# fumiama/Retrieval-based-Voice-Conversion-WebUI

Hardware: AMD Instinct MI355X
Metric: real-time factor (audio-sec/wall-sec), 48 kHz v2, 10 s clips, retrieval + NSF-HiFi-GAN decode (higher is better)
Workload: dtype fp16 MFMA operands + fp16 inter-stage streams (ResBlock outputs, ups output of stages 1-3), fp32 accumulate / in-block residual; fp32 MFMA prefilter + fp64 verified IVF distances; 1 GPU; BASELINE configs[1]: v2/48k, 1 x 10 s clip(s) per GPU, T=1198 frames, 599 queries/clip, IVF 10000x768 nlist=256 nprobe=1 k=8 index_rate=0.75; hipgraph=True, index_blob_bytes=32376576, launcher=single process

## Files before the change

retrieval-based-voice-conversion-webui_amd/csrc/mfma_conv.hpp:

```cpp
#pragma once
#include <hip/hip_runtime.h>

#include <stdint.h>

namespace rvcmi {

using bf16x8 = __attribute__((ext_vector_type(8))) __bf16;
using f16x8 = __attribute__((ext_vector_type(8))) _Float16;
using f32x16 = __attribute__((ext_vector_type(16))) float;
using f32x4 = __attribute__((ext_vector_type(4))) float;

__device__ __forceinline__ float lrelu(float v, float slope) { return v > 0.f ? v : v * slope; }

__device__ __forceinline__ int item_rows(const int* __restrict__ lens, int b, int mul, int Lmax) {
    return lens ? max(min(Lmax, lens[b] * mul), min(Lmax, mul)) : Lmax;
}


template <typename OpT>
struct Op;
template <>
struct Op<__bf16> {
    using frag = bf16x8;
    static __device__ __forceinline__ f32x16 mfma(frag a, frag b, f32x16 c) {
// ... 134 lines not shown
}
template <typename OpT, int MI>
__device__ __forceinline__ void kconv_prefetch(typename Op<OpT>::frag (&A)[8][MI], __amdgpu_buffer_rsrc_t r, unsigned loff, unsigned ctb) {
#pragma unroll
    for (int kk = 0; kk < 8; ++kk)
#pragma unroll
        for (int mi = 0; mi < MI; ++mi) A[kk][mi] = weight_load<OpT>(r, loff + kk * 1024, mi * ctb);
}
template <typename OpT, int CIN, int MI, int NJ, int STRIDE, int JT0 = 0>
__device__ __forceinline__ void kconv(f32x16 (&acc)[MI][NJ], typename Op<OpT>::frag (&A)[8][MI], unsigned lds_row, __amdgpu_buffer_rsrc_t r,
                                      unsigned loff, unsigned ctb, int ntaps, int dstep) {
    using frag = typename Op<OpT>::frag;
    constexpr int CC = CIN / 16, GPT = CC / 8;
    static_assert(CIN % 128 == 0, "kconv: C_in must be a multiple of 128");
    static_assert(JT0 >= 0 && JT0 < NJ, "kconv: at least one column tile runs");
    constexpr int NJA = NJ - JT0;
    constexpr unsigned TS = 32u * STRIDE;
    auto ld = [](unsigned a) { return *(const __attribute__((address_space(3))) frag*)(size_t)a; };
    frag Bf[2][NJ];
#pragma unroll
    for (int jt = JT0; jt < NJ; ++jt) {
        Bf[0][jt] = ld(lds_row + jt * TS);
        __builtin_amdgcn_sched_barrier(0);
    }
    const unsigned dS = (unsigned)(dstep * STRIDE);
    const int ngroups = ntaps * GPT;
    const unsigned slast = (unsigned)(ngroups - 1) * 8192u;
    unsigned soff = ngroups > 1 ? 8192u : 0u;
    int gi = 0;
    for (int g = 0; g < ngroups; ++g) {
        const unsigned nrow = (gi + 1 == GPT) ? lds_row - (unsigned)((GPT - 1) * 256) + dS : lds_row + 256u;
        unsigned b0 = lds_row, b1 = nrow;
        asm volatile("" : "+v"(b0), "+v"(b1));
#pragma unroll
        for (int kk = 0; kk < 8; ++kk) {
#pragma unroll
            for (int mi = 0; mi < MI; ++mi)
#pragma unroll
                for (int jt = JT0; jt < NJ; ++jt) {
                    constexpr int NS = MI * NJA;
                    const int i = mi * NJA + jt - JT0;
                    acc[mi][jt] = Op<OpT>::mfma(A[kk][mi], Bf[kk & 1][jt], acc[mi][jt]);
                    if (i < NJA) Bf[(kk + 1) & 1][JT0 + i] = ld((kk < 7 ? b0 + (unsigned)((kk + 1) * 32) : b1) + (JT0 + i) * TS);
                    if (i >= NS - MI) A[kk][i - (NS - MI)] = weight_load<OpT>(r, loff + kk * 1024, soff + (unsigned)(i - (NS - MI)) * ctb);
                    __builtin_amdgcn_sched_barrier(0);
                }
        }
        lds_row = nrow;
        gi = (gi + 1 == GPT) ? 0 : gi + 1;
        soff = soff < slast ? soff + 8192u : soff;
    }
}

__host__ __device__ constexpr int mfma16_row(int n) { return n < 4 ? 2 * n : n < 12 ? 2 * n - 7 : 2 * n - 16; }
__host__ __device__ constexpr int mfma16_chunk(int q) { return ((q & 1) << 1) | (q >> 1); }
__device__ __forceinline__ unsigned mfma16_loff(int lane) {
    const int q = lane >> 4, n = lane & 15;
    return (unsigned)(((q & 1) * 64 + (q >> 1) * 32 + n) * 16);
}
template <typename OpT, int MI>
__device__ __forceinline__ void kconv16_prefetch(typename Op<OpT>::frag (&A)[8][MI], __amdgpu_buffer_rsrc_t r, unsigned loff, unsigned ctb) {
    static_assert(MI == 1, "kconv16: one 32-channel tile per wave");
#pragma unroll
    for (int s = 0; s < 4; ++s)
#pragma unroll
        for (int h = 0; h < 2; ++h) A[2 * s + h][0] = weight_load<OpT>(r, loff + s * 2048 + h * 256, 0);
}
template <typename OpT, int CIN, int MI, int NJ, int STRIDE, int JT0 = 0>
__device__ __forceinline__ void kconv16(f32x4 (&acc)[2 * MI][2 * NJ], typename Op<OpT>::frag (&A)[8][MI], unsigned lds_row,
                                        __amdgpu_buffer_rsrc_t r, unsigned loff, unsigned ctb, int ntaps, int dstep) {
    using frag = typename Op<OpT>::frag;
    constexpr int CC = CIN / 16, GPT = CC / 8, NT = 2 * NJ;
    static_assert(CIN % 128 == 0, "kconv16: C_in must be a multiple of 128");
    static_assert(MI == 1, "kconv16: one 32-channel tile per wave");
    static_assert(JT0 >= 0 && JT0 < NT, "kconv16: at least one column tile runs");
    constexpr unsigned TS = 16u * STRIDE;
    auto ld = [](unsigned a) { return *(const __attribute__((address_space(3))) frag*)(size_t)a; };
    frag Bf[NT];
#pragma unroll
    for (int jt = JT0; jt < NT; ++jt) {
        Bf[jt] = ld(lds_row + jt * TS);
        __builtin_amdgcn_sched_barrier(0);
    }
    const unsigned dS = (unsigned)(dstep * STRIDE);
    const int ngroups = ntaps * GPT;
    const unsigned slast = (unsigned)(ngroups - 1) * 8192u;
    unsigned soff = ngroups > 1 ? 8192u : 0u;
    int gi = 0;
    for (int g = 0; g < ngroups; ++g) {
        const unsigned nrow = (gi + 1 == GPT) ? lds_row - (unsigned)((GPT - 1) * 256) + dS : lds_row + 256u;
        unsigned b0 = lds_row, b1 = nrow;
        asm volatile("" : "+v"(b0), "+v"(b1));
#pragma unroll
        for (int s = 0; s < 4; ++s) {
#pragma unroll
            for (int jt = JT0; jt < NT; ++jt)
#pragma unroll
                for (int h = 0; h < 2; ++h) {
                    acc[h][jt] = Op<OpT>::mfma16(A[2 * s + h][0], Bf[jt], acc[h][jt]);
                    if (h == 1) Bf[jt] = ld((s < 3 ? b0 + (unsigned)((s + 1) * 64) : b1) + jt * TS);
                    if (jt == NT - 1) A[2 * s + h][0] = weight_load<OpT>(r, loff + s * 2048 + h * 256, soff);
                    __builtin_amdgcn_sched_barrier(0);
                }
        }
        lds_row = nrow;
        gi = (gi + 1 == GPT) ? 0 : gi + 1;
// ... 84 lines not shown
```

retrieval-based-voice-conversion-webui_amd/csrc/nsf.hip:

```cpp
#include <algorithm>
#include <atomic>
#include <cmath>
#include <functional>
#include <memory>
#include <string>
#include <unordered_map>

#include "common.hpp"
#include "nsf_source_kernels.hpp"
#include "conv_kernels.hpp"
#include "post_kernels.hpp"
#include "rb_pair_kernels.hpp"
#include "ups_kernels.hpp"
#include "rb_full_kernels.hpp"
#include "conv_pack.hpp"
#include "rb_stream.hpp"

namespace rvcmi {

struct Geom {
    int MI, NJ, WCO, TT;
};
static Geom conv_geom(int cout) {
    Geom g;
// ... 104 lines not shown
            const int ctiles = (s.cout + 31) / 32;
            std::vector<uint16_t> pk((size_t)ctiles * 512, 0);
            for (int ct = 0; ct < ctiles; ++ct)
                for (int lane = 0; lane < 64; ++lane)
                    for (int e = 0; e < 8; ++e) {
                        const int co = ct * 32 + (lane & 31), kk = 8 * (lane >> 5) + e;
                        if (co < s.cout && kk < s.nk) {
                            const float v = w[(size_t)co * s.nk + kk];
                            pk[(size_t)ct * 512 + lane * 8 + e] = op == RVCMI_OPERAND_BF16 ? f32_to_bf16(v) : f32_to_f16(v);
                        }
                    }
            upload(s.nz_k1_w, pk);
            s.nz_k1 = true;
        }
    }
    s.rb.resize(cfg->n_resblock_kernels);
    for (int j = 0; j < cfg->n_resblock_kernels; ++j) {
        const int n = i * cfg->n_resblock_kernels + j;
        const int k = cfg->resblock_kernel_sizes[j];
        const int nd = cfg->n_dilations[j];
        if (nd < 1 || nd > RVCMI_MAX_DIL || !(k & 1)) RVCMI_FAIL(RVCMI_ERR_INVALID, "bad resblock %d", j);
        s.rb[j].resize(nd);
        for (int m = 0; m < nd; ++m) {
            const int d = cfg->resblock_dilation_sizes[j][m];
            const std::string base = "resblocks." + std::to_string(n);
            const int C = s.cout;
            for (int which = 0; which < 2; ++which) {
                const std::string nm = base + (which ? ".convs2." : ".convs1.") + std::to_string(m);
                const float* w = wm.get(nm + ".weight", {C, C, k});
                const float* b = wm.get(nm + ".bias", {C});
                const int dil = which ? 1 : d;
                int nt = k, off = -((k * dil - dil) / 2);
                ConvLayer& L2 = which ? s.rb[j][m].second : s.rb[j][m].first;
                build_conv(L2, C, C, 1, &nt, &off, dil,
                           [=](int co, int ci, int, int tap) { return w[((size_t)co * C + ci) * k + tap]; }, b, op);
            }
        }
    }
}

static void nsf_create(const rvcmi_nsf_config* cfg, const rvcmi_tensor* weights, int n_weights, int device, int max_B,
                       int max_T, rvcmi_nsf** out) {
    if (!cfg || !out || (!weights && n_weights)) RVCMI_FAIL(RVCMI_ERR_INVALID, "null argument");
    if (cfg->n_ups < 1 || cfg->n_ups > RVCMI_MAX_UPS || cfg->n_resblock_kernels < 1 ||
        cfg->n_resblock_kernels > RVCMI_MAX_RB)
        RVCMI_FAIL(RVCMI_ERR_INVALID, "bad stage counts");
    if (cfg->operand < 0 || cfg->operand > 2) RVCMI_FAIL(RVCMI_ERR_INVALID, "bad operand type %d", cfg->operand);
    if (max_B < 1 || max_T < 1) RVCMI_FAIL(RVCMI_ERR_INVALID, "max_B/max_T must be positive");
    HIP_CHECK(hipSetDevice(device));
    set_lds_limits();
    rb_stream_prepare();

    std::unique_ptr<rvcmi_nsf> h(new rvcmi_nsf());
    h->opt.load_env({"RB_STREAM", "NO_RB_SPLIT", "POST_DMA", "POST_DBG", "RBF_PAD_TAP", "RBF32_TALL", "DBG", "Y_F16", "X0_F16", "X0_F16_NOSTREAM"});
    rb_stream_load_env(h->opt);
    h->cfg = *cfg;
    h->device = device;
    h->max_B = max_B;
    h->max_T = max_T;
    const int op = cfg->operand;
    WeightTable wm(weights, n_weights, "nsf_create");

    const int C0 = cfg->upsample_initial_channel, inter = cfg->inter_channels;
    h->C0 = C0;
    {
        const float* w = wm.get("conv_pre.weight", {C0, inter, 7});
        const float* b = wm.get("conv_pre.bias", {C0});
        int nt = 7, off = -3;
        build_conv(h->pre, inter, C0, 1, &nt, &off, 1,
                   [=](int co, int ci, int, int tap) { return w[((size_t)co * inter + ci) * 7 + tap]; }, b, op);
    }
    if (cfg->gin_channels) {
        const float* w = wm.get("cond.weight", {C0, cfg->gin_channels, 1});
        const float* b = wm.get("cond.bias", {C0});
        upload(h->cond_w, w, (size_t)C0 * cfg->gin_channels * sizeof(float));
        upload(h->cond_b, b, C0 * sizeof(float));
    }
    if (cfg->use_f0) {
        h->lin_w = wm.get("m_source.l_linear.weight", {1, 1})[0];
        h->lin_b = wm.get("m_source.l_linear.bias", {1})[0];
    }
    int upp = 1;
    for (int i = 0; i < cfg->n_ups; ++i) upp *= cfg->upsample_rates[i];
    h->upp = upp;

    h->stages.resize(cfg->n_ups);
    size_t S = (size_t)max_T * C0;
    long L = max_T;
    for (int i = 0; i < cfg->n_ups; ++i) {
        build_stage(h->stages[i], cfg, wm, i);
        L *= h->stages[i].u;
        S = std::max(S, (size_t)L * h->stages[i].cout);
    }
    h->c_last = C0 >> cfg->n_ups;
    {
        const float* w = wm.get("conv_post.weight", {1, h->c_last, 7});
        std::vector<float> wt((size_t)7 * h->c_last);
        for (int c = 0; c < h->c_last; ++c)
            for (int j = 0; j < 7; ++j) wt[(size_t)j * h->c_last + c] = w[(size_t)c * 7 + j];
        upload(h->post_w, wt);
    }
    if (h->c_last & 3) RVCMI_FAIL(RVCMI_ERR_INVALID, "last stage channel count %d", h->c_last);

    if (cfg->n_resblock_kernels > 3) RVCMI_FAIL(RVCMI_ERR_INVALID, "more than 3 resblock kernels per stage is unsupported");
    h->S = S * (size_t)max_B;
    const size_t fb = h->S * sizeof(float);
    h->P.alloc((size_t)max_B * max_T * C0 * sizeof(float));
// ... 145 lines not shown
    }
    if (smem > 160 * 1024) RVCMI_FAIL(RVCMI_ERR_INVALID, "upsampler LDS tile too large (%zu B)", smem);
    const int per_block = WV * a.vpw;
    dim3 grid((a.Lin + TQ - 1) / TQ, (a.nvt + per_block - 1) / per_block, B);
    {
        const int esz = a.out_half ? 2 : 4;
        const size_t ot = (size_t)TQ * a.u * ((size_t)a.cout * esz + 16);
        smem = (smem + 15) / 16 * 16;
        if (a.out_tr && grid.y == 1 && (a.cout * esz) % 16 == 0 && smem + ot <= 52 * 1024) {
            a.out_tr_off = (int)smem;
            smem += ot;
        } else {
            a.out_tr = 0;
        }
    }
    if (a.out_tw_off && !a.out_tr && a.out_half && nj == 1 && MI == 2 && a.cout % 64 == 0) {
        smem = (smem + 15) / 16 * 16;
        a.out_tw_off = (int)smem;
        smem += (size_t)4 * 32 * (MI * 64 + 16);
    } else {
        a.out_tw_off = 0;
    }
    if (nj == 4) hipLaunchKernelGGL((k_ups<OpT, CIN, MI, WV, 4>), grid, dim3(256), smem, st, a);
    else if (nj == 2) hipLaunchKernelGGL((k_ups<OpT, CIN, MI, WV, 2>), grid, dim3(256), smem, st, a);
    else hipLaunchKernelGGL((k_ups<OpT, CIN, MI, WV, 1>), grid, dim3(256), smem, st, a);
}
#define RVCMI_UPS_CASES(X, OpT) \
    X(OpT, 512, 2) X(OpT, 256, 2) X(OpT, 128, 2) X(OpT, 64, 1) X(OpT, 32, 1)
template <typename OpT>
static void launch_ups_t(const UpsArgs& a, int wv, int nj, int B, hipStream_t st) {
#define X(OpT_, CIN_, MI_)                                                        \
    if (a.cin == CIN_) {                                                          \
        if (wv == 4) return launch_ups_inst<OpT_, CIN_, MI_, 4>(a, nj, B, st);    \
        if (wv == 2) return launch_ups_inst<OpT_, CIN_, MI_, 2>(a, nj, B, st);    \
        return launch_ups_inst<OpT_, CIN_, MI_, 1>(a, nj, B, st);                 \
    }
    RVCMI_UPS_CASES(X, OpT)
#undef X
    RVCMI_FAIL(RVCMI_ERR_INVALID, "unsupported upsampler C_in %d", a.cin);
}
template <typename OpT>
static void set_lds_ups() {
#define Y(OpT_, CIN_, MI_, WV_, NJ_)                                                                                    \
    HIP_CHECK(hipFuncSetAttribute(reinterpret_cast<const void*>(&k_ups<OpT_, CIN_, MI_, WV_, NJ_>),                      \
                                  hipFuncAttributeMaxDynamicSharedMemorySize, 160 * 1024));
#define X(OpT_, CIN_, MI_)                                                                                              \
    Y(OpT_, CIN_, MI_, 4, 4) Y(OpT_, CIN_, MI_, 4, 2) Y(OpT_, CIN_, MI_, 4, 1) Y(OpT_, CIN_, MI_, 2, 4) Y(OpT_, CIN_, MI_, 2, 2)   \
    Y(OpT_, CIN_, MI_, 2, 1) Y(OpT_, CIN_, MI_, 1, 4) Y(OpT_, CIN_, MI_, 1, 2) Y(OpT_, CIN_, MI_, 1, 1)
    RVCMI_UPS_CASES(X, OpT)
#undef Y
#undef X
}

template <typename OpT, int C, int MI, int NJ, int NB, int OCC, int NWV>
static void launch_rbf(size_t smem, const RbFullArgs* ra, int tiles, int nj, int B, hipStream_t st) {
    auto kern = &k_rb_full<OpT, C, MI, NJ,  4, NB, OCC, NWV>;
    if (!ra) {
        HIP_CHECK(hipFuncSetAttribute(reinterpret_cast<const void*>(kern), hipFuncAttributeMaxDynamicSharedMemorySize, 160 * 1024));
        return;
    }
    hipLaunchKernelGGL(kern, dim3(tiles, nj, B), dim3(64 * NWV), smem, st, *ra);
}
struct RbFullClass {
    int C, rows, waves;
    int MI, NJ, NB, OCC;
    size_t lds_bytes;
    void (*launch[2])(size_t, const RbFullArgs*, int, int, int, hipStream_t);
};
#define RBF_CLASS(C_, MI_, NJ_, NB_, OCC_, NWV_, STAMP_B_)                                                                     \
    {C_, NWV_ * 32 * NJ_, NWV_, MI_, NJ_, NB_, OCC_,                                                                           \
     (size_t)(2 * (NWV_ * 32 * NJ_) + 2 * RBF_G + 2 * RBF_G2) * Tile<C_>::STRIDE + 3 * 2 * 32 * MI_ * 4 + STAMP_B_,            \
     {&launch_rbf<__bf16, C_, MI_, NJ_, NB_, OCC_, NWV_>, &launch_rbf<_Float16, C_, MI_, NJ_, NB_, OCC_, NWV_>}}
static constexpr RbFullClass RBF_CLASSES[] = {
    RBF_CLASS(64, 2, 2, 2, 2, 8, 512),
    RBF_CLASS(32, 1, 3, 3, 2, 4, 512),
    RBF_CLASS(16, 1, 3, 3, 2, 4, 512),
    RBF_CLASS(64, 2, 2, 3, 1, 4, 512),
    RBF_CLASS(32, 1, 2, 3, 2, 4, 512),
    RBF_CLASS(32, 1, 3, 3, 1, 8, 1024),
};
#undef RBF_CLASS
constexpr int RBF_SMALL_ROWS = 256, RBF_TALL_ROWS = 768;
static int rbf_default_rows(int C) { return C == 64 ? 512 : 384; }
static const RbFullClass* rbf_class(int C, int rows) {
    for (const RbFullClass& c : RBF_CLASSES)
        if (c.C == C && c.rows == rows) return &c;
    RVCMI_FAIL(RVCMI_ERR_INVALID, "fused resblock: no %d-row tile class for channel count %d", rows, C);
}
static void set_lds_rbf() {
    for (const RbFullClass& c : RBF_CLASSES)
        for (auto launch : c.launch) launch(c.lds_bytes, nullptr, 0, 0, 0, nullptr);
}

static int tri_mode(const rvcmi_nsf* h, const char* key) {
    const int v = h->opt.has(key) ? h->opt.geti(key, 2) : 2;
    return v == 0 || v == 1 ? v : 2;
}
static int rbf32_tall_mode(const rvcmi_nsf* h) { return tri_mode(h, "RBF32_TALL"); }
static int rb_stream_mode(const rvcmi_nsf* h) { return tri_mode(h, "RB_STREAM"); }

static bool y_f16(const rvcmi_nsf* h) {
    return h->cfg.operand != RVCMI_OPERAND_F32 && h->opt.geti("Y_F16", 1) != 0;
}

static void run_conv(rvcmi_nsf* h, const ConvLayer& L, ConvArgs a, int B, const char* name, hipStream_t st) {
    if (!a.cf_stride) a.cf_stride = a.Lin;
    a.cin = L.cin;
    a.cout = L.cout;
    a.bias = L.bias.as<float>();
    a.dstep = L.dstep;
    a.nphase = L.nphase;
    const int op = h->cfg.operand;
    int jsum = 0;
    for (int p = 0; p < L.nphase; ++p) {
        a.ph_in_off[p] = L.in_off[p];
        a.ph_ntaps[p] = L.ntaps[p];
        a.ph_w_off[p] = op == RVCMI_OPERAND_F32 ? L.f32_off[p] : L.pack_off[p];
        jsum += L.ntaps[p];
    }
    a.in_off = L.in_off[0];
    const double flops = L.flops_per_pos * (double)a.Lq * B;
    const size_t esz = op == RVCMI_OPERAND_F32 ? 4 : 2;
    double bytes = (double)B * a.Lin * L.cin * (a.in_mode == IN_OP_RAW ? esz : 4) +
                   (double)B * a.Lq * L.nphase * L.cout * (a.out_mode == OUT_ACT ? esz : 4) * (a.accumulate ? 2 : 1) +
                   (a.res ? (double)B * a.Lq * L.nphase * L.cout * 4 : 0) + (double)jsum * L.cin * L.cout * esz;
    if (op == RVCMI_OPERAND_F32) {
        a.w = L.w_f32.p;
        a.ntaps = L.ntaps[0];
        a.roff = 0;
        a.tile_rows = 0;
        const size_t n = (size_t)a.Lq * a.cout;
        dim3 grid((unsigned)((n + 255) / 256), L.nphase, B);
        h->prof.launch(name, flops, bytes, st, [&] { hipLaunchKernelGGL(k_conv_f32, grid, dim3(256), 0, st, a); });
    } else {
        Geom g = conv_geom(L.cout);
        int nj = 4;
        if (g.MI == 2 && g.WCO == 4 && (long)B * ((a.Lq + g.TT - 1) / g.TT) * ((L.cout + 255) / 256) * L.nphase < 128) {
            nj = 1;
            g.TT = 32;
        }
        a.w = L.w_pack.p;
        a.w_ct_stride = L.ct_stride;
        a.ntaps = L.ntaps_p;
        const int span = (L.ntaps_p - 1) * std::abs(L.dstep);
        a.roff = L.dstep < 0 ? span : 0;
// ... 552 lines not shown
        const RbStreamJob& J = p.stream.args.job[j];
        r.k[j] = J.k;
        r.tiles[j] = J.nstrips;
        r.strip_len[j] = J.strip_len;
        src[j] = h->Ya[j].as<float>();
    }
}

static void rb_full(const Fwd& f, const Stage& s, const StagePlan& p, long L, int lm, const float** src) {
    rvcmi_nsf* h = f.h;
    const int C = s.cout, nk = (int)s.rb.size(), B = f.B;
    char nm[48];
    snprintf(nm, sizeof(nm), "rb_full_c%d", C);
    RbFullArgs ra;
    memset(&ra, 0, sizeof(ra));
    ra.L = (int)L;
    ra.lens = f.lens;
    ra.lmul = lm;
    ra.bstride = L * C;
    ra.dbg = dbg_flags(h);
    ra.yh = p.stage_half ? 1 : 0;
    ra.xh = p.x0_half ? 1 : 0;
    ra.pad_tap = h->opt.geti("RBF_PAD_TAP", 0) != 0 ? 1 : 0;
    const int R = p.full->rows;
    rvcmi_nsf_stage_plan& r = *f.rec;
    r.tile_rows = R;
    r.tile_waves = p.full->waves;
    r.n_rb = nk;
    int order[RVCMI_MAX_RB];
    rb_order(s, order);
    int max_tiles = 0;
    double flops = 0, bytes = 0;
    for (int oj = 0; oj < nk; ++oj) {
        const int j = order[oj];
        RbFullJob& J = ra.job[oj];
        J.src = h->X0.as<float>();
        J.dst = h->Ya[j].as<float>();
        J.nd = (int)s.rb[j].size();
        fill_rb_job(J, s.rb[j], 0, J.nd, L, B, C, flops, bytes);
        for (int m = 0; m < J.nd; ++m)
            if (J.dil[m] * (J.k - 1) / 2 + J.dil[m] > RBF_G) RVCMI_FAIL(RVCMI_ERR_INVALID, "dilation too large for the fused resblock");
        J.HL = rbf_halo(s.rb[j]);
        J.tvalid = R - 2 * J.HL;
        if (J.tvalid < R / 4) RVCMI_FAIL(RVCMI_ERR_INVALID, "resblock halo too large for the fused kernel");
        J.ntiles = (int)((L + J.tvalid - 1) / J.tvalid);
        max_tiles = std::max(max_tiles, J.ntiles);
        r.k[oj] = J.k;
        r.tiles[oj] = J.ntiles;
        bytes += (double)B * L * C * ((p.stage_half ? 2 : 4) + (p.x0_half ? 2 : 4));
        src[j] = J.dst;
    }
    const size_t nblk = (size_t)max_tiles * nk * B;
    if (ra.dbg & 32) ra.ts = stamp_buffer(h, nblk * 8 * 16, f.st);
    h->prof.launch(nm, flops, bytes, f.st, [&] { p.full->launch[f.op == RVCMI_OPERAND_BF16 ? 0 : 1](p.full->lds_bytes, &ra, max_tiles, nk, B, f.st); });
    HIP_CHECK(hipGetLastError());
    if (ra.dbg & 32) print_stamps(h, nm, ra, nk, max_tiles, p.full->waves, 16, nblk, f.st);
}

static void rb_pair(const Fwd& f, const Stage& s, long L, int lm, const float** src) {
    rvcmi_nsf* h = f.h;
    const int op = f.op, C = s.cout, nk = (int)s.rb.size(), B = f.B;
    const int mode = rb_stream_mode(h);
    char nm[48], nms[48];
    snprintf(nm, sizeof(nm), "rb_pair_c%d", C);
    snprintf(nms, sizeof(nms), "rb_stream1_c%d", C);
    int order[RVCMI_MAX_RB];
    rb_order(s, order);
    rvcmi_nsf_stage_plan& r = *f.rec;
    r.tile_rows = rb_rows(C);
    for (size_t m = 0; m < max_levels(s); ++m) {
        RbPairArgs ra;
        memset(&ra, 0, sizeof(ra));
        ra.lens = f.lens;
        ra.lmul = lm;
        ra.L = (int)L;
        ra.bstride = L * C;
        ra.dbg = dbg_flags(h);
        RbStreamDesc sd[RVCMI_MAX_RB];
        float* dsts[RVCMI_MAX_RB] = {nullptr};
        int nj = 0, max_tiles = 0, max_rows = 0;
        double flops = 0, bytes = 0;
        for (int oj = 0; oj < nk; ++oj) {
            const int j = order[oj];
            if (m >= s.rb[j].size()) continue;
            RbStreamDesc& d = sd[nj];
            memset(&d, 0, sizeof(d));
            d.src = src[j];
            d.dst = dsts[j] = ydst(h, j, m);
            d.lens = f.lens;
            d.lmul = lm;
            fill_rb_job(d, s.rb[j], (int)m, 1, L, B, C, flops, bytes);
            bytes += (double)B * L * C * 8;
            RbJob& J = ra.job[nj++];
            J.src = d.src; J.dst = d.dst; J.w1 = d.w1[0]; J.w2 = d.w2[0]; J.b1 = d.b1[0]; J.b2 = d.b2[0];
            J.ct1 = d.ct1; J.ct2 = d.ct2; J.k = d.k; J.k_p = d.k_p; J.dil = d.dil[0];
            J.tt2 = rb_rows(C) - (J.k - 1);
            J.ntiles = (int)((L + J.tt2 - 1) / J.tt2);
            max_tiles = std::max(max_tiles, J.ntiles);
            max_rows = std::max(max_rows, rb_rows(C) + (J.k_p - 1) * J.dil);
            if (m == 0) {
                r.k[r.n_rb] = J.k;
                r.tiles[r.n_rb++] = J.ntiles;
            }
        }
        constexpr int NWp = 8;
        const size_t nblk = (size_t)max_tiles * nj * B;
        if (ra.dbg & 32) ra.ts = stamp_buffer(h, nblk * NWp * 8, f.st);
// ... 93 lines not shown
        for (auto& v : src) v = h->X0.as<float>();
        switch (p.path) {
            case RbPath::F32_CHAIN: rb_f32_chain(f, s, L, lm, src); break;
            case RbPath::SPLIT: rb_split(f, s, L, lm, src); break;
            case RbPath::STREAM: rb_stream(f, s, p, src); break;
            case RbPath::FULL: rb_full(f, s, p, L, lm, src); break;
            case RbPath::PAIR: rb_pair(f, s, L, lm, src); break;
        }
        const int nk = (int)s.rb.size();
        a = Act{{src[0], nk > 1 ? src[1] : nullptr, nk > 2 ? src[2] : nullptr}, p.stage_half, false, (float)nk, L, C, lm};
        snprintf(nm, sizeof(nm), "stage%d", i);
        if (f.want(nm)) return tap_stage(f, a);
    }
    if (tr) RVCMI_FAIL(RVCMI_ERR_INVALID, "unknown tap '%s'", tr->what);
    conv_post(f, a, out);
}

}

extern "C" {

int rvcmi_nsf_create(const rvcmi_nsf_config* cfg, const rvcmi_tensor* weights, int n_weights, int device, int max_B,
                     int max_T, rvcmi_nsf** out) {
    return guarded([&] { nsf_create(cfg, weights, n_weights, device, max_B, max_T, out); });
}
int rvcmi_nsf_destroy(rvcmi_nsf* h) {
    return guarded([&] { delete h; });
}
int rvcmi_nsf_forward(rvcmi_nsf* h, int B, int T, const int* lengths, const float* x, const float* f0, const float* g,
                      const float* noise, int n_res, float* out, void* stream) {
    return guarded([&] { nsf_forward(h, B, T, lengths, x, f0, g, noise, n_res, out, (hipStream_t)stream, nullptr); });
}
int rvcmi_nsf_upp(const rvcmi_nsf* h) { return h ? h->upp : RVCMI_ERR_INVALID; }
size_t rvcmi_nsf_workspace_bytes(const rvcmi_nsf* h) { return h ? h->ws_bytes : 0; }

int rvcmi_nsf_debug_forward(rvcmi_nsf* h, int B, int T, const float* x, const float* f0, const float* g,
                            const float* noise, int n_res, const char* what, float* out_host, size_t capacity_floats,
                            int64_t shape_out[3], void* stream) {
    return guarded([&] {
        if (!what || !out_host || !shape_out) RVCMI_FAIL(RVCMI_ERR_INVALID, "null argument");
        TapRequest tr;
        tr.what = what;
        tr.out_host = out_host;
        tr.capacity = capacity_floats;
        tr.shape = shape_out;
        nsf_forward(h, B, T, nullptr, x, f0, g, noise, n_res, nullptr, (hipStream_t)stream, &tr);
        if (!tr.done) RVCMI_FAIL(RVCMI_ERR_INVALID, "tap '%s' was not produced", what);
    });
}

int rvcmi_nsf_set_option(rvcmi_nsf* h, const char* key, double value) {
    return guarded([&] {
        if (!h || !key) RVCMI_FAIL(RVCMI_ERR_INVALID, "null argument");
        if ((!strcmp(key, "RBF_PAD_TAP") || !strcmp(key, "RBF32_TALL")) && value == value && value != 0.0 && value != 1.0)
            RVCMI_FAIL(RVCMI_ERR_INVALID, "option '%s' takes 0 or 1", key);
        if (!strcmp(key, "RS_MFMA") && value == value && value != 16.0 && value != 32.0) RVCMI_FAIL(RVCMI_ERR_INVALID, "option 'RS_MFMA' takes 16 or 32");
        if (!h->opt.set(key, value)) RVCMI_FAIL(RVCMI_ERR_INVALID, "unknown option '%s' for this handle", key);
    });
}
int rvcmi_nsf_profile_enable(rvcmi_nsf* h, int enable) {
    return guarded([&] {
        if (!h) RVCMI_FAIL(RVCMI_ERR_INVALID, "null handle");
        h->prof.enabled = enable != 0;
    });
}
int rvcmi_nsf_last_plan(const rvcmi_nsf* h, rvcmi_nsf_stage_plan* out, int capacity, int* n) {
    return guarded([&] {
        if (!h || !n || (!out && h->n_plan)) RVCMI_FAIL(RVCMI_ERR_INVALID, "null argument");
        if (capacity < h->n_plan) RVCMI_FAIL(RVCMI_ERR_INVALID, "capacity %d for the %d stages of the last forward", capacity, h->n_plan);
        std::copy(h->last_plan, h->last_plan + h->n_plan, out);
        *n = h->n_plan;
    });
}
int rvcmi_nsf_profile_read(rvcmi_nsf* h, rvcmi_kernel_stat* stats, int capacity, int* n, int reset) {
    return guarded([&] {
        if (!h) RVCMI_FAIL(RVCMI_ERR_INVALID, "null handle");
        h->prof.read(stats, capacity, n, reset);
    });
}

}
```

retrieval-based-voice-conversion-webui_amd/csrc/rb_full_kernels.hpp:

```cpp
#pragma once
#include <hip/hip_runtime.h>

#include "mfma_conv.hpp"

namespace rvcmi {

struct RbFullJob {
    const float* src;
    float* dst;
    const void* w1[3];
    const void* w2[3];
    const float* b1[3];
    const float* b2[3];
    long ct1, ct2;
    int k, k_p;
    int dil[3];
    int nd;
    int HL;
    int tvalid;
    int ntiles;
};
struct RbFullArgs {
    RbFullJob job[3];
    int L;
    const int* lens;
    int lmul;
    long bstride;
    int dbg;
    int yh;
    int xh;
    unsigned long long* ts;
    int pad_tap;
};

constexpr int RBF_G = 32;
constexpr int RBF_G2 = 8;

template <typename OpT, int C, int MI, int NJ, int KG, int NB, int OCC = 1, int NWV = 4>
static __global__ void __launch_bounds__(64 * NWV, OCC) k_rb_full(RbFullArgs a) {
    constexpr int NT = 64 * NWV;
    using TL = Tile<C>;
    constexpr int STRIDE = TL::STRIDE;
    constexpr int SLAB = 32 * NJ;
    constexpr int R = NWV * SLAB;
    constexpr int XROWS = R + 2 * RBF_G;
    constexpr int HROWS = R + 2 * RBF_G2;
    constexpr int CP = 32 * MI;
    extern __shared__ __attribute__((aligned(16))) char smem[];
    char* X = smem;
    char* H = smem + (size_t)XROWS * STRIDE;
    float* bias_l = (float*)(smem + (size_t)(XROWS + HROWS) * STRIDE);
    unsigned long long* tsl = (unsigned long long*)(bias_l + 3 * 2 * CP);

    const RbFullJob& J = a.job[blockIdx.y];
    if ((int)blockIdx.x >= J.ntiles) return;
    const int b = blockIdx.z;
    const int Lb = item_rows(a.lens, b, a.lmul, a.L);
    const int tg0 = blockIdx.x * J.tvalid - J.HL;
    if (tg0 + J.HL >= Lb) return;
    const float* src = J.src + (size_t)b * a.bstride;
    float* dst = J.dst + (size_t)b * a.bstride;
    const int wave = threadIdx.x >> 6, lane = threadIdx.x & 63;
    const int slab = wave * SLAB;
    const int half4 = 4 * (lane >> 5);

    int tsn = 0;
    auto stamp = [&]() {
#ifdef RVCMI_DEV_STAMPS
        if ((a.dbg & 32) && lane == 0 && tsn < 16) tsl[wave * 16 + tsn] = __builtin_readcyclecounter();
#endif
        ++tsn;
    };
    stamp();

    const bool interior = tg0 >= 0 && tg0 + R <= Lb;
    unsigned rowmask[NJ];
#pragma unroll
    for (int jt = 0; jt < NJ; ++jt) {
        const int tg = tg0 + slab + jt * 32 + (lane & 31);
        rowmask[jt] = (tg >= 0 && tg < Lb) ? 0xffffffffu : 0u;
    }

    constexpr bool TIO = C % 32 == 0;
    constexpr int TS = C * 4 + 16;
    constexpr int C4 = C / 4;
    static_assert(!TIO || (size_t)R * TS <= (size_t)(XROWS + HROWS) * STRIDE, "transposition tile must fit the X | H regions");
    static_assert(!TIO || (R * C4) % NT == 0, "whole batches of row chunks");
    f32x16 xacc[MI][NJ];
    if (a.xh) {
        const _Float16* srch = (const _Float16*)J.src + (size_t)b * a.bstride;
        if constexpr (TIO) {
// ... 70 lines not shown
        }
        __syncthreads();
#pragma unroll
        for (int mi = 0; mi < MI; ++mi)
#pragma unroll
            for (int jt = 0; jt < NJ; ++jt)
#pragma unroll
                for (int g = 0; g < 4; ++g) {
                    const f32x4 q = *(const f32x4*)(smem + (size_t)(slab + jt * 32 + (lane & 31)) * TS + (mi * 32 + 8 * g + half4) * 4);
#pragma unroll
                    for (int e = 0; e < 4; ++e) xacc[mi][jt][4 * g + e] = q[e];
                }
        __syncthreads();
    } else
#pragma unroll
    for (int mi = 0; mi < MI; ++mi)
#pragma unroll
        for (int jt = 0; jt < NJ; ++jt) {
            const int tg = tg0 + slab + jt * 32 + (lane & 31);
            const int tgc = min(max(tg, 0), Lb - 1);
#pragma unroll
            for (int g = 0; g < 4; ++g) {
                if (mi * 32 + 8 * g < C) {
                    const f32x4 v = *(const f32x4*)(src + (size_t)tgc * C + mi * 32 + 8 * g + half4);
#pragma unroll
                    for (int e = 0; e < 4; ++e) xacc[mi][jt][4 * g + e] = mask_bits(v[e], rowmask[jt]);
                } else {
#pragma unroll
                    for (int e = 0; e < 4; ++e) xacc[mi][jt][4 * g + e] = 0.f;
                }
            }
        }
    {
        constexpr int W = STRIDE / 16;
        const uint4 z = make_uint4(0, 0, 0, 0);
        for (int i = threadIdx.x; i < 2 * RBF_G * W; i += NT) {
            const int r = i / W, c = i - r * W;
            const int row = r < RBF_G ? r : RBF_G + R + (r - RBF_G);
            *(uint4*)(X + (size_t)row * STRIDE + c * 16) = z;
        }
        for (int i = threadIdx.x; i < 2 * RBF_G2 * W; i += NT) {
            const int r = i / W, c = i - r * W;
            const int row = r < RBF_G2 ? r : RBF_G2 + R + (r - RBF_G2);
            *(uint4*)(H + (size_t)row * STRIDE + c * 16) = z;
        }
        for (int i = threadIdx.x; i < J.nd * 2 * CP; i += NT) {
            const int m = i / (2 * CP), w = (i / CP) & 1, c = i % CP;
            const float* bp = w ? J.b2[m] : J.b1[m];
            bias_l[i] = c < C ? bp[c] : 0.f;
        }
    }

    stamp();
    typename Op<OpT>::frag A[NB][KG][MI];
    conv_prefetch<OpT, C, MI, KG, NB>(A, (const OpT*)J.w1[0] + lane * 8, J.ct1, J.k_p);
    char* xw = X + (size_t)(RBF_G + slab + (lane & 31)) * STRIDE + half4 * 2;
    char* hw = H + (size_t)(RBF_G2 + slab + (lane & 31)) * STRIDE + half4 * 2;
    publish_operand<OpT, C, MI, NJ, STRIDE, false>(xw, xacc, rowmask);
    stamp();
    __syncthreads();
    stamp();

    const char* xl = X + (size_t)(slab + (lane & 31)) * STRIDE + (lane >> 5) * 16;
    const char* hl = H + (size_t)(slab + (lane & 31)) * STRIDE + (lane >> 5) * 16;
    const int p2 = (J.k - 1) / 2;
    constexpr bool REAL = TL::CC < KG;
    const int nks = (REAL && !a.pad_tap ? J.k : J.k_p) * TL::CC;

    for (int m = 0; m < J.nd; ++m) {
        const int p1 = J.dil[m] * (J.k - 1) / 2;
        f32x16 hacc[MI][NJ];
        {
            const float* bl = bias_l + (m * 2 + 0) * CP + half4;
#pragma unroll
            for (int mi = 0; mi < MI; ++mi)
#pragma unroll
                for (int g = 0; g < 4; ++g) {
                    const f32x4 bv = *(const f32x4*)(bl + mi * 32 + 8 * g);
#pragma unroll
                    for (int jt = 0; jt < NJ; ++jt)
#pragma unroll
                        for (int e = 0; e < 4; ++e) hacc[mi][jt][4 * g + e] = bv[e];
                }
        }
        conv_run<OpT, C, MI, NJ, KG, NB, REAL>(hacc, A, xl, (const OpT*)J.w1[m] + lane * 8, J.ct1, J.k_p, RBF_G - p1, J.dil[m], nks);
        conv_prefetch<OpT, C, MI, KG, NB>(A, (const OpT*)J.w2[m] + lane * 8, J.ct2, J.k_p);
        if (m == 0) stamp();
        if (interior) publish_operand<OpT, C, MI, NJ, STRIDE, false>(hw, hacc, rowmask);
        else publish_operand<OpT, C, MI, NJ, STRIDE, true>(hw, hacc, rowmask);
        if (m == 0) stamp();
        __syncthreads();
        if (m == 0) stamp();
        {
            const float* bl = bias_l + (m * 2 + 1) * CP + half4;
#pragma unroll
            for (int mi = 0; mi < MI; ++mi)
#pragma unroll
                for (int g = 0; g < 4; ++g) {
                    const f32x4 bv = *(const f32x4*)(bl + mi * 32 + 8 * g);
#pragma unroll
                    for (int jt = 0; jt < NJ; ++jt)
#pragma unroll
                        for (int e = 0; e < 4; ++e) xacc[mi][jt][4 * g + e] += bv[e];
                }
        }
        conv_run<OpT, C, MI, NJ, KG, NB, REAL>(xacc, A, hl, (const OpT*)J.w2[m] + lane * 8, J.ct2, J.k_p, RBF_G2 - p2, 1, nks);
        if (m + 1 < J.nd) conv_prefetch<OpT, C, MI, KG, NB>(A, (const OpT*)J.w1[m + 1] + lane * 8, J.ct1, J.k_p);
        if (m == 0) stamp();
        if (m + 1 < J.nd) {
            if (interior) publish_operand<OpT, C, MI, NJ, STRIDE, false>(xw, xacc, rowmask);
            else publish_operand<OpT, C, MI, NJ, STRIDE, true>(xw, xacc, rowmask);
            if (m == 0) stamp();
            __syncthreads();
            if (m == 0) stamp();
        }
    }
    stamp();

    if (a.yh) {
        _Float16* dsth = (_Float16*)J.dst + (size_t)b * a.bstride;
        if constexpr (TIO) {
            constexpr int TSH = C * 2 + 16;
            constexpr int C8 = C / 8;
            __syncthreads();
#pragma unroll
            for (int mi = 0; mi < MI; ++mi)
#pragma unroll
                for (int jt = 0; jt < NJ; ++jt)
#pragma unroll
                    for (int g = 0; g < 4; ++g)
                        *(uint2*)(smem + (size_t)(slab + jt * 32 + (lane & 31)) * TSH + (mi * 32 + 8 * g + half4) * 2) =
                            pack4_h(xacc[mi][jt][4 * g + 0], xacc[mi][jt][4 * g + 1], xacc[mi][jt][4 * g + 2], xacc[mi][jt][4 * g + 3]);
            __syncthreads();
            if (!(a.dbg & 16)) {
                const int nrow = min(R - 2 * J.HL, Lb - (tg0 + J.HL));
                const int tot = nrow * C8;
                for (int i = threadIdx.x; i < tot; i += NT) {
                    const int r = i / C8, c8 = i - r * C8;
                    const int row = J.HL + r;
                    *(uint4*)(dsth + (size_t)(tg0 + row) * C + c8 * 8) = *(const uint4*)(smem + (size_t)row * TSH + c8 * 16);
                }
            }
        } else if (!(a.dbg & 16)) {
#pragma unroll
            for (int mi = 0; mi < MI; ++mi)
#pragma unroll
                for (int jt = 0; jt < NJ; ++jt) {
                    const int row = slab + jt * 32 + (lane & 31);
                    const int tg = tg0 + row;
                    if (row >= J.HL && row < R - J.HL && tg < Lb) {
#pragma unroll
                        for (int g = 0; g < 4; ++g)
                            if (mi * 32 + 8 * g < C)
                                *(uint2*)(dsth + (size_t)tg * C + mi * 32 + 8 * g + half4) =
                                    pack4_h(xacc[mi][jt][4 * g + 0], xacc[mi][jt][4 * g + 1], xacc[mi][jt][4 * g + 2], xacc[mi][jt][4 * g + 3]);
                    }
                }
        }
    } else if constexpr (TIO) {
        __syncthreads();
// ... 48 lines not shown
```

Before: 5930 x real-time (audio-sec/wall-sec), whole job.

## Add lean k-loop ring conv path for small-channel fused ResBlock kernels

```diff
diff --git a/retrieval-based-voice-conversion-webui_amd/csrc/mfma_conv.hpp b/retrieval-based-voice-conversion-webui_amd/csrc/mfma_conv.hpp
--- a/retrieval-based-voice-conversion-webui_amd/csrc/mfma_conv.hpp
+++ b/retrieval-based-voice-conversion-webui_amd/csrc/mfma_conv.hpp
@@ -210,6 +210,67 @@
     }
 }
 
+template <typename OpT, int CIN, int MI, int NJ, int STRIDE, bool TAIL>
+__device__ __forceinline__ void kconv_small_ring(f32x16 (&acc)[MI][NJ], typename Op<OpT>::frag (&A)[8][MI], typename Op<OpT>::frag (&Bf)[2][NJ],
+                                                 unsigned lds_row, unsigned dS, __amdgpu_buffer_rsrc_t r, unsigned loff, unsigned ctb, unsigned slo,
+                                                 unsigned shi, int rem) {
+    using frag = typename Op<OpT>::frag;
+    constexpr int CC = CIN / 16, TPR = 8 / CC;
+    constexpr unsigned TS = 32u * STRIDE;
+    auto ld = [](unsigned a) { return *(const __attribute__((address_space(3))) frag*)(size_t)a; };
+    unsigned b[TPR + 1];
+#pragma unroll
+    for (int j = 0; j <= TPR; ++j) {
+        b[j] = lds_row + (unsigned)j * dS;
+        asm volatile("" : "+v"(b[j]));
+    }
+#pragma unroll
+    for (int kk = 0; kk < 8; ++kk) {
+        if constexpr (TAIL)
+            if (kk > 0 && kk % CC == 0 && kk >= rem) return;
+        const unsigned nb = b[(kk + 1) / CC] + (unsigned)(((kk + 1) % CC) * 32);
+#pragma unroll
+        for (int mi = 0; mi < MI; ++mi)
+#pragma unroll
+            for (int jt = 0; jt < NJ; ++jt) {
+                constexpr int NS = MI * NJ;
+                const int i = mi * NJ + jt;
+                acc[mi][jt] = Op<OpT>::mfma(A[kk][mi], Bf[kk & 1][jt], acc[mi][jt]);
+                if (i < NJ) Bf[(kk + 1) & 1][i] = ld(nb + i * TS);
+                if constexpr (!TAIL)
+                    if (i >= NS - MI) A[kk][i - (NS - MI)] = weight_load<OpT>(r, loff + (kk & 3) * 1024, (kk < 4 ? slo : shi) + (unsigned)(i - (NS - MI)) * ctb);
+                __builtin_amdgcn_sched_barrier(0);
+            }
+    }
+}
+template <typename OpT, int CIN, int MI, int NJ, int STRIDE>
+__device__ __forceinline__ void kconv_small(f32x16 (&acc)[MI][NJ], typename Op<OpT>::frag (&A)[8][MI], unsigned lds_row, __amdgpu_buffer_rsrc_t r,
+                                            unsigned loff, unsigned ctb, int nkp, int nrun, int dstep) {
+    using frag = typename Op<OpT>::frag;
+    static_assert(CIN == 64 || CIN == 32, "kconv_small: C_in = 64 or 32 (8 k-steps = 2 or 4 whole taps, at least 8 packed k-steps per conv)");
+    constexpr int TPR = 8 / (CIN / 16);
+    constexpr unsigned TS = 32u * STRIDE;
+    auto ld = [](unsigned a) { return *(const __attribute__((address_space(3))) frag*)(size_t)a; };
+    frag Bf[2][NJ];
+#pragma unroll
+    for (int jt = 0; jt < NJ; ++jt) {
+        Bf[0][jt] = ld(lds_row + jt * TS);
+        __builtin_amdgcn_sched_barrier(0);
+    }
+    const unsigned dS = (unsigned)(dstep * STRIDE);
+    const unsigned smax = (unsigned)(nkp - 4) * 1024u;
+    unsigned slo = min(8192u, smax), shi = min(8192u + 4096u, smax);
+    const int nfull = nrun >> 3;
+    for (int g = 0; g < nfull; ++g) {
+        kconv_small_ring<OpT, CIN, MI, NJ, STRIDE, false>(acc, A, Bf, lds_row, dS, r, loff, ctb, slo, shi, 8);
+        lds_row += (unsigned)TPR * dS;
+        slo = min(slo + 8192u, smax);
+        shi = min(shi + 8192u, smax);
+    }
+    const int rem = nrun & 7;
+    if (rem) kconv_small_ring<OpT, CIN, MI, NJ, STRIDE, true>(acc, A, Bf, lds_row, dS, r, loff, ctb, 0u, 0u, rem);
+}
+
 __host__ __device__ constexpr int mfma16_row(int n) { return n < 4 ? 2 * n : n < 12 ? 2 * n - 7 : 2 * n - 16; }
 __host__ __device__ constexpr int mfma16_chunk(int q) { return ((q & 1) << 1) | (q >> 1); }
 __device__ __forceinline__ unsigned mfma16_loff(int lane) {
diff --git a/retrieval-based-voice-conversion-webui_amd/csrc/nsf.hip b/retrieval-based-voice-conversion-webui_amd/csrc/nsf.hip
--- a/retrieval-based-voice-conversion-webui_amd/csrc/nsf.hip
+++ b/retrieval-based-voice-conversion-webui_amd/csrc/nsf.hip
@@ -180,7 +180,7 @@
     rb_stream_prepare();
 
     std::unique_ptr<rvcmi_nsf> h(new rvcmi_nsf());
-    h->opt.load_env({"RB_STREAM", "NO_RB_SPLIT", "POST_DMA", "POST_DBG", "RBF_PAD_TAP", "RBF32_TALL", "DBG", "Y_F16", "X0_F16", "X0_F16_NOSTREAM"});
+    h->opt.load_env({"RB_STREAM", "NO_RB_SPLIT", "POST_DMA", "POST_DBG", "RBF_PAD_TAP", "RBF32_TALL", "RBF_KL", "DBG", "Y_F16", "X0_F16", "X0_F16_NOSTREAM"});
     rb_stream_load_env(h->opt);
     h->cfg = *cfg;
     h->device = device;
@@ -432,9 +432,9 @@
 #undef X
 }
 
-template <typename OpT, int C, int MI, int NJ, int NB, int OCC, int NWV>
+template <typename OpT, int C, int MI, int NJ, int NB, int OCC, int NWV, int KL>
 static void launch_rbf(size_t smem, const RbFullArgs* ra, int tiles, int nj, int B, hipStream_t st) {
-    auto kern = &k_rb_full<OpT, C, MI, NJ,  4, NB, OCC, NWV>;
+    auto kern = &k_rb_full<OpT, C, MI, NJ,  4, NB, OCC, NWV, KL>;
     if (!ra) {
         HIP_CHECK(hipFuncSetAttribute(reinterpret_cast<const void*>(kern), hipFuncAttributeMaxDynamicSharedMemorySize, 160 * 1024));
         return;
@@ -446,11 +446,15 @@
     int MI, NJ, NB, OCC;
     size_t lds_bytes;
     void (*launch[2])(size_t, const RbFullArgs*, int, int, int, hipStream_t);
+    void (*lean[2])(size_t, const RbFullArgs*, int, int, int, hipStream_t);
 };
 #define RBF_CLASS(C_, MI_, NJ_, NB_, OCC_, NWV_, STAMP_B_)                                                                     \
     {C_, NWV_ * 32 * NJ_, NWV_, MI_, NJ_, NB_, OCC_,                                                                           \
      (size_t)(2 * (NWV_ * 32 * NJ_) + 2 * RBF_G + 2 * RBF_G2) * Tile<C_>::STRIDE + 3 * 2 * 32 * MI_ * 4 + STAMP_B_,            \
-     {&launch_rbf<__bf16, C_, MI_, NJ_, NB_, OCC_, NWV_>, &launch_rbf<_Float16, C_, MI_, NJ_, NB_, OCC_, NWV_>}}
+     {&launch_rbf<__bf16, C_, MI_, NJ_, NB_, OCC_, NWV_, 0>, &launch_rbf<_Float16, C_, MI_, NJ_, NB_, OCC_, NWV_, 0>}, RBF_LEAN_##C_(MI_, NJ_, NB_, OCC_, NWV_)}
+#define RBF_LEAN_64(MI_, NJ_, NB_, OCC_, NWV_) {&launch_rbf<__bf16, 64, MI_, NJ_, NB_, OCC_, NWV_, 1>, &launch_rbf<_Float16, 64, MI_, NJ_, NB_, OCC_, NWV_, 1>}
+#define RBF_LEAN_32(MI_, NJ_, NB_, OCC_, NWV_) {&launch_rbf<__bf16, 32, MI_, NJ_, NB_, OCC_, NWV_, 1>, &launch_rbf<_Float16, 32, MI_, NJ_, NB_, OCC_, NWV_, 1>}
+#define RBF_LEAN_16(MI_, NJ_, NB_, OCC_, NWV_) {nullptr, nullptr}
 static constexpr RbFullClass RBF_CLASSES[] = {
     RBF_CLASS(64, 2, 2, 2, 2, 8, 512),
     RBF_CLASS(32, 1, 3, 3, 2, 4, 512),
@@ -460,6 +464,9 @@
     RBF_CLASS(32, 1, 3, 3, 1, 8, 1024),
 };
 #undef RBF_CLASS
+#undef RBF_LEAN_64
+#undef RBF_LEAN_32
+#undef RBF_LEAN_16
 constexpr int RBF_SMALL_ROWS = 256, RBF_TALL_ROWS = 768;
 static int rbf_default_rows(int C) { return C == 64 ? 512 : 384; }
 static const RbFullClass* rbf_class(int C, int rows) {
@@ -469,8 +476,12 @@
 }
 static void set_lds_rbf() {
     for (const RbFullClass& c : RBF_CLASSES)
-        for (auto launch : c.launch) launch(c.lds_bytes, nullptr, 0, 0, 0, nullptr);
-}
+        for (int op = 0; op < 2; ++op) {
+            c.launch[op](c.lds_bytes, nullptr, 0, 0, 0, nullptr);
+            if (c.lean[op]) c.lean[op](c.lds_bytes, nullptr, 0, 0, 0, nullptr);
+        }
+}
+static bool rbf_lean(const rvcmi_nsf* h, const RbFullClass& c) { return c.lean[0] && h->opt.geti("RBF_KL", 1) != 0; }
 
 static int tri_mode(const rvcmi_nsf* h, const char* key) {
     const int v = h->opt.has(key) ? h->opt.geti(key, 2) : 2;
@@ -1129,7 +1140,10 @@
     }
     const size_t nblk = (size_t)max_tiles * nk * B;
     if (ra.dbg & 32) ra.ts = stamp_buffer(h, nblk * 8 * 16, f.st);
-    h->prof.launch(nm, flops, bytes, f.st, [&] { p.full->launch[f.op == RVCMI_OPERAND_BF16 ? 0 : 1](p.full->lds_bytes, &ra, max_tiles, nk, B, f.st); });
+    bool lean = rbf_lean(h, *p.full);
+    for (int oj = 0; oj < nk; ++oj) lean = lean && ra.job[oj].k_p * (C / 16) >= 8;
+    const auto launch = (lean ? p.full->lean : p.full->launch)[f.op == RVCMI_OPERAND_BF16 ? 0 : 1];
+    h->prof.launch(nm, flops, bytes, f.st, [&] { launch(p.full->lds_bytes, &ra, max_tiles, nk, B, f.st); });
     HIP_CHECK(hipGetLastError());
     if (ra.dbg & 32) print_stamps(h, nm, ra, nk, max_tiles, p.full->waves, 16, nblk, f.st);
 }
@@ -1329,7 +1343,7 @@
 int rvcmi_nsf_set_option(rvcmi_nsf* h, const char* key, double value) {
     return guarded([&] {
         if (!h || !key) RVCMI_FAIL(RVCMI_ERR_INVALID, "null argument");
-        if ((!strcmp(key, "RBF_PAD_TAP") || !strcmp(key, "RBF32_TALL")) && value == value && value != 0.0 && value != 1.0)
+        if ((!strcmp(key, "RBF_PAD_TAP") || !strcmp(key, "RBF32_TALL") || !strcmp(key, "RBF_KL")) && value == value && value != 0.0 && value != 1.0)
             RVCMI_FAIL(RVCMI_ERR_INVALID, "option '%s' takes 0 or 1", key);
         if (!strcmp(key, "RS_MFMA") && value == value && value != 16.0 && value != 32.0) RVCMI_FAIL(RVCMI_ERR_INVALID, "option 'RS_MFMA' takes 16 or 32");
         if (!h->opt.set(key, value)) RVCMI_FAIL(RVCMI_ERR_INVALID, "unknown option '%s' for this handle", key);
diff --git a/retrieval-based-voice-conversion-webui_amd/csrc/rb_full_kernels.hpp b/retrieval-based-voice-conversion-webui_amd/csrc/rb_full_kernels.hpp
--- a/retrieval-based-voice-conversion-webui_amd/csrc/rb_full_kernels.hpp
+++ b/retrieval-based-voice-conversion-webui_amd/csrc/rb_full_kernels.hpp
@@ -36,7 +36,7 @@
 constexpr int RBF_G = 32;
 constexpr int RBF_G2 = 8;
 
-template <typename OpT, int C, int MI, int NJ, int KG, int NB, int OCC = 1, int NWV = 4>
+template <typename OpT, int C, int MI, int NJ, int KG, int NB, int OCC = 1, int NWV = 4, int KL = 0>
 static __global__ void __launch_bounds__(64 * NWV, OCC) k_rb_full(RbFullArgs a) {
     constexpr int NT = 64 * NWV;
     using TL = Tile<C>;
@@ -213,8 +213,11 @@
     }
 
     stamp();
-    typename Op<OpT>::frag A[NB][KG][MI];
-    conv_prefetch<OpT, C, MI, KG, NB>(A, (const OpT*)J.w1[0] + lane * 8, J.ct1, J.k_p);
+    typename Op<OpT>::frag A[KL ? 1 : NB][KG][MI];
+    typename Op<OpT>::frag A8[8][MI];
+    const unsigned loff = lane * 16, ctb1 = (unsigned)(J.ct1 * sizeof(OpT)), ctb2 = (unsigned)(J.ct2 * sizeof(OpT));
+    if constexpr (KL) kconv_prefetch<OpT, MI>(A8, weight_rsrc(J.w1[0]), loff, ctb1);
+    else conv_prefetch<OpT, C, MI, KG, NB>(A, (const OpT*)J.w1[0] + lane * 8, J.ct1, J.k_p);
     char* xw = X + (size_t)(RBF_G + slab + (lane & 31)) * STRIDE + half4 * 2;
     char* hw = H + (size_t)(RBF_G2 + slab + (lane & 31)) * STRIDE + half4 * 2;
     publish_operand<OpT, C, MI, NJ, STRIDE, false>(xw, xacc, rowmask);
@@ -227,6 +230,7 @@
     const int p2 = (J.k - 1) / 2;
     constexpr bool REAL = TL::CC < KG;
     const int nks = (REAL && !a.pad_tap ? J.k : J.k_p) * TL::CC;
+    const int nkp = J.k_p * TL::CC;
 
     for (int m = 0; m < J.nd; ++m) {
         const int p1 = J.dil[m] * (J.k - 1) / 2;
@@ -244,8 +248,13 @@
                         for (int e = 0; e < 4; ++e) hacc[mi][jt][4 * g + e] = bv[e];
                 }
         }
-        conv_run<OpT, C, MI, NJ, KG, NB, REAL>(hacc, A, xl, (const OpT*)J.w1[m] + lane * 8, J.ct1, J.k_p, RBF_G - p1, J.dil[m], nks);
-        conv_prefetch<OpT, C, MI, KG, NB>(A, (const OpT*)J.w2[m] + lane * 8, J.ct2, J.k_p);
+        if constexpr (KL) {
+            kconv_small<OpT, C, MI, NJ, STRIDE>(hacc, A8, lds_address(xl + (RBF_G - p1) * STRIDE), weight_rsrc(J.w1[m]), loff, ctb1, nkp, nks, J.dil[m]);
+            kconv_prefetch<OpT, MI>(A8, weight_rsrc(J.w2[m]), loff, ctb2);
+        } else {
+            conv_run<OpT, C, MI, NJ, KG, NB, REAL>(hacc, A, xl, (const OpT*)J.w1[m] + lane * 8, J.ct1, J.k_p, RBF_G - p1, J.dil[m], nks);
+            conv_prefetch<OpT, C, MI, KG, NB>(A, (const OpT*)J.w2[m] + lane * 8, J.ct2, J.k_p);
+        }
         if (m == 0) stamp();
         if (interior) publish_operand<OpT, C, MI, NJ, STRIDE, false>(hw, hacc, rowmask);
         else publish_operand<OpT, C, MI, NJ, STRIDE, true>(hw, hacc, rowmask);
@@ -265,8 +274,13 @@
                         for (int e = 0; e < 4; ++e) xacc[mi][jt][4 * g + e] += bv[e];
                 }
         }
-        conv_run<OpT, C, MI, NJ, KG, NB, REAL>(xacc, A, hl, (const OpT*)J.w2[m] + lane * 8, J.ct2, J.k_p, RBF_G2 - p2, 1, nks);
-        if (m + 1 < J.nd) conv_prefetch<OpT, C, MI, KG, NB>(A, (const OpT*)J.w1[m + 1] + lane * 8, J.ct1, J.k_p);
+        if constexpr (KL) {
+            kconv_small<OpT, C, MI, NJ, STRIDE>(xacc, A8, lds_address(hl + (RBF_G2 - p2) * STRIDE), weight_rsrc(J.w2[m]), loff, ctb2, nkp, nks, 1);
+            if (m + 1 < J.nd) kconv_prefetch<OpT, MI>(A8, weight_rsrc(J.w1[m + 1]), loff, ctb1);
+        } else {
+            conv_run<OpT, C, MI, NJ, KG, NB, REAL>(xacc, A, hl, (const OpT*)J.w2[m] + lane * 8, J.ct2, J.k_p, RBF_G2 - p2, 1, nks);
+            if (m + 1 < J.nd) conv_prefetch<OpT, C, MI, KG, NB>(A, (const OpT*)J.w1[m + 1] + lane * 8, J.ct1, J.k_p);
+        }
         if (m == 0) stamp();
         if (m + 1 < J.nd) {
             if (interior) publish_operand<OpT, C, MI, NJ, STRIDE, false>(xw, xacc, rowmask);
```

New measurement: 6015 x real-time (audio-sec/wall-sec), whole job, median of 3. +1.4%, better.
